# featureform/embeddinghub

Measured on AMD Instinct MI355X. Metric: kNN queries/sec at recall@10>=0.95, 10Mx768 cosine, batch=1024, higher is better.
Workload: dtype i8 filter -> f32 exact results; 1 GPU; 10000000x768 cosine (EHX-GAUSS-1), batch=1024, k=10, exact scan; rows=10000000, dims=768, batch=1024, k=10, rows_dtype=f32, world_size=1, parallelism=single GPU

## Files before the change

embeddinghub_amd/csrc/ehx_flat.cpp:

```cpp
#include "ehx_internal.h"

namespace ehx_impl {

ScanPlan plan_scan(uint32_t nq, uint32_t n_tiles, uint32_t k, int n_cus) {
  ScanPlan p;
  p.q_tiles = (nq + kTileQ - 1) / kTileQ;
  p.q_rows = p.q_tiles * kTileQ;
  p.n_tiles = n_tiles;
  p.kprime = k + 8;
  uint32_t chunks = (uint32_t)n_cus / p.q_tiles;
  if (chunks < 1) chunks = 1;
  if (chunks >= 8) chunks &= ~7u;
  if (chunks > p.n_tiles) chunks = p.n_tiles ? p.n_tiles : 1;
  p.n_chunks = chunks;
  p.tiles_per_chunk = p.n_tiles ? (p.n_tiles + chunks - 1) / chunks : 0;
  p.grid = p.q_tiles * p.n_chunks;
  p.xcd_map = (p.n_chunks % 8 == 0) ? 1u : 0u;
  return p;
}

std::vector<ScanPass> plan_cascade(uint32_t nq, uint32_t n_tiles, uint32_t k, int n_cus, uint64_t first_tiles, uint64_t growth) {
  std::vector<ScanPass> passes;
  uint64_t done = 0;
  for (uint64_t cum = first_tiles; cum * 2 < n_tiles; cum *= growth) {
// ... 60 lines not shown
                                  s->scr.dQgamma.p, s->scr.dQuv.p, st));
  if (n_pub == 0) {
    HIP_TRY(hipMemsetAsync(s->scr.dMerged.p, 0xFF, (size_t)p.q_rows * 64 * sizeof(uint64_t), st));
    if ((rc = clock.scan_begin(st)) || (rc = clock.scan_end(st))) return rc;
  } else {
    auto cascade = [&](auto& a, auto launch) -> int {
      for (size_t i = 0; i < passes.size(); ++i) {
        const bool last = i + 1 == passes.size();
        set_scan_pass(a, passes[i].plan, passes[i].tile0);
        HIP_TRY(launch(a, st));
        if (last && (rc = clock.scan_end(st))) return rc;
        HIP_TRY(launch_flat_merge(s->scr.dPart.p, (uint32_t)nq, passes[i].plan.n_chunks * lpc, p.kprime, s->scr.dMerged.p, st,
                                  lists_total, i > 0, last ? nullptr : (unsigned long long*)s->scr.dGthr.p));
      }
      return EHX_OK;
    };
    HIP_TRY(hipMemsetAsync(s->scr.dGthr.p, 0xFF, (size_t)p.q_rows * sizeof(uint64_t), st));
    if ((rc = clock.scan_begin(st))) return rc;
    if (f16) {
      ScanArgs16 h;
      scan_args_shared(h, s->scr.dCand.p, s->scr.dPart.p, s->scr.dScanErr.p, s->scr.dGthr.p, p, lists_total, n_pub);
      h.Q = s->scr.dQ16.p;
      h.X = s->f16.dX16.p;
      h.rowp = s->f16.dRowp16.p;
      h.qgamma = s->scr.dQgamma.p;
      h.eps = scan16_eps(s->dims);
      h.cos = s->metric == EHX_METRIC_COSINE;
      h.ld = s->ld16;
      if (sample) {
        ScanPlan sp = plan_scan((uint32_t)nq, kSampleTiles, k, E.n_cus);
        set_scan_pass(h, sp, 0);
        h.dump = s->scr.dSample.p;
        HIP_TRY(launch_flat_scan16(h, st));
        h.dump = nullptr;
        HIP_TRY(launch_sample_select(s->scr.dSample.p, kSampleTiles * kTileRows16, p.q_rows, (uint32_t)nq, p.kprime,
                                     (unsigned long long*)s->scr.dGthr.p, st));
      }
      if ((rc = cascade(h, launch_flat_scan16))) return rc;
    } else {
      ScanArgs a;
      scan_args_shared(a, s->scr.dCand.p, s->scr.dPart.p, s->scr.dScanErr.p, s->scr.dGthr.p, p, lists_total, n_pub);
      a.Q = s->scr.dQ.p;
      a.X = s->rows.dX.p;
      a.x_half = (uint32_t)s->x_half;
      a.rowp = s->rows.dRowp.p;
      a.ld = s->ld;
      if ((rc = cascade(a, launch_flat_scan8))) return rc;
    }
  }
  RerankArgs r;
  r.Q = s->scr.dQ.p;
  r.rows = rows_view(s, n_pub);
  r.merged = s->scr.dMerged.p;
  r.out_ids = d_ids;
  r.out_dist = d_dist;
  r.out_count = d_count;
  r.n_uncertified = s->scr.verdict.count.p;
  r.nq = (uint32_t)nq;
  r.k = k;
  r.kprime = p.kprime;
  if (f16) r.quv = s->scr.dQuv.p;
  r.max_sumsq = s->rows.dMaxSumsq.p;
  r.uncert_flags = s->scr.verdict.flags.p;
  HIP_TRY(launch_rerank(r, st));
  if ((rc = clock.finish(st))) return rc;
  s->n_rerank += (uint64_t)nq * p.kprime;
  return EHX_OK;
}

int resolve_engine(const ehx_space* s, uint64_t n_pub) {
  if (s->params.mode != EHX_MODE_FLAT || s->scan_sel == EHX_SCAN_F32 || n_pub == 0) return EHX_ENGINE_F32;
  if (s->scan_sel == EHX_SCAN_AUTO && s->has8 && s->h_unsafe8.load(std::memory_order_relaxed) == 0 && n_pub >= s->i8_min_rows)
    return EHX_ENGINE_I8;
  if (s->has16 && s->h_unsafe.load(std::memory_order_relaxed) == 0) return EHX_ENGINE_F16;
  return EHX_ENGINE_F32;
}

static int i8_diagnose(ehx_space::I8Set::Buffers& b, hipStream_t st, size_t nq, uint32_t k, uint32_t width,
                       const uint32_t* d_ovf, const float* d_dist) {
  HIP_TRY(hipStreamSynchronize(st));
  if (env().i8_count) {
    unsigned long long c[8] = {0};
    HIP_TRY(hipMemcpy(c, b.dCnt.p, sizeof(c), hipMemcpyDeviceToHost));
    fprintf(stderr, "[i8 count] tests %llu alarms %llu row-block alarms %llu trips %llu (cumulative)\n", c[0], c[1], c[2], c[3]);
  }
  if (env().i8_debug) {
    std::vector<uint32_t> fl(nq), ov(nq);
    std::vector<float4> qp(nq);
    std::vector<float2> uv(nq);
    std::vector<uint64_t> mg(nq * width);
    std::vector<float> od(nq * k);
    HIP_TRY(hipMemcpy(fl.data(), b.verdict.flags.p, nq * 4, hipMemcpyDeviceToHost));
    HIP_TRY(hipMemcpy(ov.data(), d_ovf, nq * 4, hipMemcpyDeviceToHost));
    HIP_TRY(hipMemcpy(qp.data(), b.dQp8.p, nq * sizeof(float4), hipMemcpyDeviceToHost));
    HIP_TRY(hipMemcpy(uv.data(), b.dQuv.p, nq * sizeof(float2), hipMemcpyDeviceToHost));
    HIP_TRY(hipMemcpy(mg.data(), b.dMerged8.p, nq * width * 8, hipMemcpyDeviceToHost));
    HIP_TRY(hipMemcpy(od.data(), d_dist, nq * k * 4, hipMemcpyDeviceToHost));
    int shown = 0;
    for (size_t q = 0; q < nq && shown < 6; ++q) {
      if (!fl[q]) continue;
      ++shown;
      auto S = [&](int i) { return mg[q * width + i] == ~0ull ? INFINITY : ordered_to_f32((uint32_t)(mg[q * width + i] >> 32)); };
      fprintf(stderr, "[i8 debug] q=%zu ovf=%u tmin=%g S[0]=%g S[63]=%g S[127]=%g S[255]=%g kth_dist=%g u=%g v=%g\n", q, ov[q],
              qp[q].w, S(0), S(63), S(127), S(255), od[q * k + k - 1], uv[q].x, uv[q].y);
    }
  }
  return EHX_OK;
}

static int flat_pass8(ehx_space* s, uint64_t n_pub, int set, hipStream_t st, size_t nq, const float* d_queries, uint32_t k,
                      uint64_t* d_ids, float* d_dist, uint32_t* d_count, uint32_t* kprime_used) {
  Engine& E = engine();
  ehx_space::I8Set& sc = s->i8set[set];
  const uint32_t n_tiles = (uint32_t)((n_pub + kTileRows16 - 1) / kTileRows16);
  const bool big = n_tiles >= 2048;
  const uint32_t growth = env().i8_growth ? env().i8_growth : (big ? 8u : 4u);
  const double safety = [] {
    return env().i8_safety;
  }();
  const int sync_mode = env().i8_sync;
  const bool use_sync = sync_mode > 0;
  constexpr uint32_t kSampleTiles = 8;
  const uint32_t width = s->i8_width.load(std::memory_order_relaxed);
  const long kprime_env = env().i8_kprime;
  uint32_t kp_auto = n_pub >= 4000000 ? 256u : 128u;
  if (s->dims <= 128) kp_auto = 64u;
  else if (s->dims < 512) kp_auto = 128u;
  if (s->dims >= 1024) kp_auto = width;
  const uint32_t kp_want = std::max(kp_auto, s->i8_kprime_min.load(std::memory_order_relaxed));
  const uint32_t kprime = kprime_env >= 64 ? (uint32_t)std::min<long>(kprime_env, (long)width) : std::min(kp_want, width);
  s->i8_kprime_last.store(kprime, std::memory_order_relaxed);
  *kprime_used = kprime;
  const uint32_t kFirstTiles = env().i8_first_tiles ? env().i8_first_tiles : (big ? 128u : 512u);
  const std::vector<ScanPass> passes = plan_cascade((uint32_t)nq, n_tiles, k, E.n_cus, kFirstTiles, growth);
  auto rank_after = [&](size_t i) -> uint32_t {
    if (i + 1 >= passes.size()) return kprime;
    const double f = (double)((uint64_t)(passes[i + 1].tile0) * kTileRows16) / (double)n_pub;
    return (uint32_t)std::min<double>(kprime, std::max<double>(16.0, std::ceil(kprime * f * safety)));
  };
  const uint64_t first_rows = (uint64_t)passes.front().plan.n_tiles * kTileRows16;
  const uint64_t first_keys_env = env().i8_first_keys;
  const uint64_t first_floor = first_keys_env ? first_keys_env : (big ? 64ull : std::min<uint64_t>(512, 2ull * kprime));
  const uint64_t first_keys = std::min<uint64_t>(
      2048, passes.size() == 1 ? 2ull * kprime : std::max<uint64_t>(first_floor, 2ull * rank_after(0)));
  const uint32_t sample_rank =
      (uint32_t)std::min<uint64_t>(64, std::max<uint64_t>(8, first_keys * kSampleTiles * kTileRows16 / first_rows));
  const ScanPlan p = passes.back().plan;
  test_pause();
  uint32_t grid_max = 0, chunks_max = 0;
  for (auto& ps : passes) {
    grid_max = std::max(grid_max, ps.plan.grid);
    chunks_max = std::max(chunks_max, ps.plan.n_chunks);
  }
  if (chunks_max > 256) return fail(EHX_EINTERNAL, "scan plan with %u chunks", chunks_max);
  int rc;
  ScanArgsI8 a;
  if ((rc = i8_scan_args(s, sc.buf, p, n_pub, &a))) return rc;
  if ((rc = sc.buf.dSample8.ensure((size_t)kSampleTiles * kTileRows16 * p.q_rows))) return rc;
  if ((rc = sc.buf.dMerged8.ensure((size_t)p.q_rows * width))) return rc;
  if ((rc = sc.buf.verdict.ensure(p.q_rows, ehx_space::I8Set::kStampWords))) return rc;
  constexpr uint32_t kTable = kBalanceMaxChunks + 1;
  std::vector<int> stamp_slot(passes.size(), -1);
  sc.n_stamped = 0;
  if (s->ld8 % 256u == 0u && !s->keyless) {
    const uint32_t min_tpc = s->i8_balance_min_tpc.load(std::memory_order_relaxed);
    uint32_t off = 0;
    for (size_t i = passes.size(); i-- > 0 && sc.n_stamped < ehx_space::I8Set::kStampedPasses;) {
// ... 334 lines not shown
```

embeddinghub_amd/csrc/k_flati8.hip:

```cpp
#include "ehx_env.h"
#include "ehx_kernels.h"
#include "k_scan_common.h"

namespace ehx {

typedef int i32x4 __attribute__((ext_vector_type(4)));

namespace {

constexpr uint32_t kRingI8 = 4;
constexpr uint32_t kRowBI8 = 64;
constexpr uint32_t kStageI8 = kTileRows16 * kRowBI8;
template <bool HALF>
struct I8L {
  static constexpr int kThreads = HALF ? 256 : 512;
  static constexpr uint32_t kWaves = HALF ? 4 : 8;
  static constexpr uint32_t kXStage = HALF ? kStageI8 / 2 : kStageI8;
  static constexpr uint32_t kXShift = HALF ? 13 : 14;
  static constexpr uint32_t kQSlots = HALF ? 2 : kRingI8;
  static constexpr uint32_t kStgCap = HALF ? 64 : 128;
  static constexpr uint32_t kRowpSlot = (HALF ? 128 : 256) * 16;
  static constexpr uint32_t kRowpWaves = HALF ? 2 : 4;
  static constexpr uint32_t kXOff = 0;
  static constexpr uint32_t kQOff = kRingI8 * kXStage;
  static constexpr uint32_t kRowpOff = kQOff + kQSlots * kStageI8;
  static constexpr uint32_t kQpOff = kRowpOff + 3 * kRowpSlot;
  static constexpr uint32_t kQinvOff = kQpOff + kTileQ * 16;
  static constexpr uint32_t kSyncOff = kQinvOff + kTileQ * 4;
  static constexpr uint32_t kCtxOff = kSyncOff + 256;
  static constexpr uint32_t kStgKeyOff = kCtxOff + 64;
  static constexpr uint32_t kStgQlOff = kStgKeyOff + kWaves * kStgCap * 8;
  static constexpr uint32_t kStgCntOff = kStgQlOff + kWaves * kStgCap * 4;
  static constexpr uint32_t kLdsBytes = kStgCntOff + 64;
};
static_assert(I8L<false>::kLdsBytes <= 160 * 1024, "LDS budget");
static_assert(I8L<true>::kLdsBytes <= 80 * 1024, "LDS budget: two half-tile workgroups per CU");
static_assert(I8L<false>::kQOff == 64 * 1024 && I8L<false>::kRowpOff == 128 * 1024, "layout of the full-tile kernel");
static_assert(kTileRows16 == 256 && kTileQ == 256, "kernel geometry is hard-wired");

#define EHX_MFMA_I8(A, B, C) __builtin_amdgcn_mfma_i32_16x16x64_i8((A), (B), (C), 0, 0, 0)

#ifndef EHX_I8_ABL
#define EHX_I8_ABL 0
#endif
#ifndef EHX_I8_COUNT
#define EHX_I8_COUNT 0
#endif
#ifndef EHX_I8_PRIO
#define EHX_I8_PRIO 1
#endif
#if EHX_I8_COUNT
#define EHX_CNT(I) do { if (lane == 0) atomicAdd((unsigned long long*)a.cand + (I), 1ull); } while (0)
#else
#define EHX_CNT(I) do { } while (0)
#endif

__device__ __forceinline__ void lds_barrier_i8() {
  __builtin_amdgcn_s_waitcnt(0xC07F);
  __builtin_amdgcn_s_barrier();
}

__device__ __forceinline__ float i8_score(const float4 P, const float4 qq, int v) {
  const float t = qq.x * (float)v;
  const float K = __builtin_fmaf(P.y, qq.z, __builtin_fmaf(P.z, qq.y, P.w));
  return __builtin_fmaf(P.x, t, K);
}

__device__ __forceinline__ float i8_alarm_k(const float4 tp, const float4 qq, const float qinv) {
  const float bg = tp.w * qq.z, ce = tp.y * qq.y;
  float num = bg - tp.z - ce - qq.w;
  num -= 1e-5f * (fabsf(bg) + tp.z + ce + fabsf(qq.w));
  if (!(num > 0.0f)) return -__builtin_inff();
  return num * qinv;
}

struct I8Ctx {
  uint64_t* pool;
  uint32_t* pool_cnt;
  uint32_t* ovf;
  const uint8_t* perm;
  const float4* rowp;
  uint32_t pool_cap;
  uint32_t n;
  uint32_t q_tile0;
  uint32_t allow_bits;
  const uint32_t* allow;
};
static_assert(sizeof(I8Ctx) <= 64, "I8Ctx slot");

constexpr int kMaskNone = 0, kMaskOne = 1, kMaskPerQuery = 2, kMaskLabel = 3;
template <bool HALF, int MASKED>
__device__ __attribute__((noinline)) void i8_flush_staging() {
  using L = I8L<HALF>;
  extern __shared__ __attribute__((aligned(16))) char smem[];
  const I8Ctx* ctx = (const I8Ctx*)(smem + L::kCtxOff);
  const int lane = threadIdx.x & 63, w = threadIdx.x >> 6;
  const uint64_t* keys = (const uint64_t*)(smem + L::kStgKeyOff) + (size_t)w * L::kStgCap;
  const uint32_t* qls = (const uint32_t*)(smem + L::kStgQlOff) + (size_t)w * L::kStgCap;
  const float4* qp_lds = (const float4*)(smem + L::kQpOff);
  uint32_t* cnt = (uint32_t*)(smem + L::kStgCntOff) + w;
  uint32_t n = *cnt;
  if (n > L::kStgCap) n = L::kStgCap;
  const uint32_t cap = ctx->pool_cap;
  for (uint32_t i = (uint32_t)lane; i < n; i += 64) {
    const uint64_t e = keys[i];
    const uint32_t posn = (uint32_t)e;
    const int v = (int)(uint32_t)(e >> 32);
    const uint32_t qloc = (uint32_t)(w & 3) * 64u + qls[i];
    const float4 qq = qp_lds[qloc];
    const float S = i8_score(ctx->rowp[posn], qq, v);
    if (!(S <= qq.w) || posn >= ctx->n) continue;
    const uint32_t id = (posn & 0xFFFFFF00u) | (uint32_t)ctx->perm[posn];
    if constexpr (MASKED == kMaskOne) {
      if (id >= ctx->allow_bits || !((ctx->allow[id >> 5] >> (id & 31u)) & 1u)) continue;
    }
    if constexpr (MASKED == kMaskPerQuery) {
      if (id >= ctx->allow_bits) continue;
      const uint32_t* block = ctx->allow;
      if (!((block[(size_t)block[ctx->q_tile0 + qloc] + (id >> 5)] >> (id & 31u)) & 1u)) continue;
    }
    if constexpr (MASKED == kMaskLabel) {
      if (id >= ctx->allow_bits) continue;
      const uint32_t* block = ctx->allow;
      if (block[(size_t)kLabelHead + id] != block[ctx->q_tile0 + qloc]) continue;
    }
    const uint64_t key = ((uint64_t)f32_to_ordered(S) << 32) | (uint64_t)id;
    const uint32_t q = ctx->q_tile0 + qloc;
    const uint32_t pos = atomicAdd(&ctx->pool_cnt[q], 1u);
    if (pos < cap) ctx->pool[(size_t)q * cap + pos] = key;
    else ctx->ovf[q] = 1u;
  }
  asm volatile("s_waitcnt vmcnt(0) lgkmcnt(0)" ::: "memory");
  if (lane == 0) *cnt = 0u;
  asm volatile("s_waitcnt lgkmcnt(0)" ::: "memory");
}

template <bool HALF, int MASKED>
__device__ __forceinline__ void i8_hit(int v, bool hi, uint32_t r_local, uint32_t tile_row0, int ql, int w, uint32_t& stg_n) {
  using L = I8L<HALF>;
  extern __shared__ __attribute__((aligned(16))) char smem[];
  const uint64_t m = __ballot(hi);
  if (m == 0ull) return;
  const uint32_t k = (uint32_t)__builtin_popcountll(m);
  uint32_t* cnt = (uint32_t*)(smem + L::kStgCntOff) + w;
  if (stg_n + k > L::kStgCap) {
    if ((threadIdx.x & 63) == 0) *cnt = stg_n;
    asm volatile("s_waitcnt lgkmcnt(0)" ::: "memory");
    i8_flush_staging<HALF, MASKED>();
    stg_n = 0u;
  }
  if (hi) {
    const uint32_t pos = stg_n + __builtin_amdgcn_mbcnt_hi((uint32_t)(m >> 32), __builtin_amdgcn_mbcnt_lo((uint32_t)m, 0u));
    uint64_t* keys = (uint64_t*)(smem + L::kStgKeyOff) + (size_t)w * L::kStgCap;
    uint32_t* qls = (uint32_t*)(smem + L::kStgQlOff) + (size_t)w * L::kStgCap;
    keys[pos] = ((uint64_t)(uint32_t)v << 32) | (uint64_t)(tile_row0 + r_local);
    qls[pos] = (uint32_t)ql;
  }
  stg_n += k;
}

}

size_t scan_i8_lds_bytes() { return I8L<false>::kLdsBytes; }

template <bool DUMP, bool REV, bool QRES = false, bool HALF = false, bool PAIR = false, int MASKED = kMaskNone, bool TAB = false>
__global__ __launch_bounds__(I8L<HALF>::kThreads, 2) void flat_scan_i8_kernel(const ScanArgsI8 a) {
  static_assert(!TAB || (REV && !DUMP && !QRES && !HALF && !PAIR && !MASKED), "TAB: the plain compile-time-slot scan only");
  static_assert(!QRES || (!REV && !DUMP), "QRES: the run-time-slot loop of the plain scan only");
  static_assert(!PAIR || (!REV && !DUMP && !QRES && !HALF), "PAIR: the run-time-slot loop of the plain scan, stages in pairs");
  static_assert(!HALF || QRES, "HALF: short rows, the query tile resident in LDS");
  static_assert(!MASKED || !DUMP, "MASKED: the flush of a collecting scan");
  using L = I8L<HALF>;
  extern __shared__ __attribute__((aligned(16))) char smem[];
  const int tid = threadIdx.x;
  const int lane = tid & 63;
  const int w = __builtin_amdgcn_readfirstlane(tid >> 6);
  const int j15 = lane & 15, qd = lane >> 4;

  uint32_t qt, chunk, half = 0u;
  {
    uint32_t b = blockIdx.x;
    if (a.xcd_map) {
      const uint32_t xcd = b & 7u;
      uint32_t slot = b >> 3;
      if constexpr (HALF) {
        half = slot & 1u;
        slot >>= 1;
      }
      qt = slot % a.q_tiles;
      chunk = xcd * (a.n_chunks >> 3) + slot / a.q_tiles;
    } else {
      if constexpr (HALF) {
        half = b & 1u;
        b >>= 1;
      }
      qt = b % a.q_tiles;
      chunk = b / a.q_tiles;
    }
    half = (uint32_t)__builtin_amdgcn_readfirstlane((int)half);
    qt = (uint32_t)__builtin_amdgcn_readfirstlane((int)qt);
    chunk = (uint32_t)__builtin_amdgcn_readfirstlane((int)chunk);
  }
  const int wr = HALF ? (int)half : (w >> 2), wc = w & 3;
  const uint32_t lrow0 = HALF ? 0u : (uint32_t)wr * 128u;
  float4* qp_lds = (float4*)(smem + L::kQpOff);
  float* qinv_lds = (float*)(smem + L::kQinvOff);

  if (tid < (int)kTileQ) {
    const size_t qg = (size_t)qt * kTileQ + tid;
    float4 qp = a.qparams[qg];
    qp.w = a.thr ? a.thr[qg] : __builtin_inff();
    qp_lds[tid] = qp;
    qinv_lds[tid] = qp.x > 0.0f ? (1.0f - 1e-5f) / qp.x : __builtin_inff();
  }
  if (tid < 64) ((uint32_t*)(smem + L::kSyncOff))[tid] = 0u;
  if (tid < 8) ((uint32_t*)(smem + L::kStgCntOff))[tid] = 0u;
  if (tid == 0) {
    I8Ctx* ctx = (I8Ctx*)(smem + L::kCtxOff);
    ctx->pool = a.pool;
    ctx->pool_cnt = a.pool_cnt;
    ctx->ovf = a.ovf;
    ctx->perm = a.perm;
    ctx->rowp = a.rowp;
    ctx->pool_cap = a.pool_cap;
    ctx->n = a.n;
    ctx->q_tile0 = qt * kTileQ;
    ctx->allow_bits = MASKED ? a.allow_bits : 0u;
    if constexpr (MASKED) ctx->allow = a.allow;
  }

  uint32_t tile_begin = a.tile0 + chunk * a.tiles_per_chunk;
  uint32_t tile_end = tile_begin + a.tiles_per_chunk;
  if (tile_end > a.tile0 + a.n_tiles) tile_end = a.tile0 + a.n_tiles;
  if constexpr (TAB) {
    if (a.bounds) {
      typedef const __attribute__((address_space(4))) uint32_t* cu32p;
      const uint64_t bv = (uint64_t)(a.bounds + chunk);
      const uint32_t blo = (uint32_t)__builtin_amdgcn_readfirstlane((int)(uint32_t)bv);
      const uint32_t bhi = (uint32_t)__builtin_amdgcn_readfirstlane((int)(uint32_t)(bv >> 32));
      const cu32p bp = (cu32p)(((uint64_t)bhi << 32) | blo);
      tile_begin = a.tile0 + bp[0];
      tile_end = a.tile0 + bp[1];
      if (tile_end > a.tile0 + a.n_tiles) tile_end = a.tile0 + a.n_tiles;
      if (tile_begin > tile_end) tile_begin = tile_end;
    }
  }
  const uint32_t my_tiles =
      (uint32_t)__builtin_amdgcn_readfirstlane((int)(tile_end > tile_begin ? tile_end - tile_begin : 0u));
  const uint32_t ktiles = a.ld / kRowBI8;

  const uint32_t voff = (uint32_t)lane * 16u;
  const uint32_t voff8 = voff + L::kXStage / 2;
  const size_t tile_bytes = (size_t)ktiles * kStageI8;
  const char* xsrc = (const char*)a.X + (size_t)tile_begin * tile_bytes + (size_t)half * L::kXStage * (HALF ? 1u : 0u) +
                     (size_t)w * 1024;
  const char* qbase = (const char*)a.Q + (size_t)qt * ((size_t)(ktiles + 3) * kStageI8) + (size_t)w * 1024;
  const char* qsrc = qbase;
  const uint32_t rpiece = (uint32_t)w & (L::kRowpWaves - 1u);
  const char* rsrc = (const char*)(a.rowp + (size_t)tile_begin * kTileRows16 + (HALF ? (size_t)half * 128u : 0u)) +
                     (size_t)rpiece * 1024;
  const uint32_t xdst = L::kXOff + (uint32_t)w * 1024u;
  const uint32_t qdst = L::kQOff + (uint32_t)w * 1024u;
  const uint32_t rdst = L::kRowpOff + rpiece * 1024u;

#define EHX_DMA(DST_BASE, DST_IMM, VOFF, SRC)                                                              \
  do {                                                                                                     \
    asm volatile("s_add_u32 m0, %0, %1\n\ts_nop 0\n\tglobal_load_lds_dwordx4 %2, %3"                       \
                 :                                                                                         \
                 : "s"(DST_BASE), "n"(DST_IMM), "v"(VOFF), "s"(SRC)                                        \
                 : "memory", "scc");                                                                       \
  } while (0)
#define EHX_DMA_RT(DST, VOFF, SRC)                                                       \
  do {                                                                                   \
    asm volatile("s_mov_b32 m0, %0\n\ts_nop 0\n\tglobal_load_lds_dwordx4 %1, %2"         \
                 :                                                                       \
                 : "s"(DST), "v"(VOFF), "s"(SRC)                                         \
                 : "memory");                                                            \
  } while (0)
#define EHX_DMA_X0(SLOT) EHX_DMA(xdst, (SLOT) * L::kXStage, voff, xsrc)
#define EHX_DMA_Q0(SLOT) EHX_DMA(qdst, (SLOT) * 16384, voff, qsrc)
#define EHX_DMA_X1(SLOT) EHX_DMA(xdst, (SLOT) * L::kXStage + L::kXStage / 2, voff8, xsrc)
#define EHX_DMA_Q1(SLOT)                               \
  do {                                                 \
    EHX_DMA(qdst, (SLOT) * 16384 + 8192, voff8, qsrc);  \
    xsrc += kStageI8;                                  \
    qsrc += kStageI8;                                  \
  } while (0)

  const uint32_t sw = scan8_swz((uint32_t)j15);
  uint32_t a_off = L::kXOff + (lrow0 + (uint32_t)j15) * kRowBI8 + (((uint32_t)qd) ^ sw) * 16u;
  uint32_t b_off = L::kQOff + (uint32_t)(wc * 64 + j15) * kRowBI8 + (((uint32_t)qd) ^ sw) * 16u;
  asm volatile("" : "+v"(a_off), "+v"(b_off));

  i32x4 acc[8][4];
#pragma unroll
  for (int rb = 0; rb < 8; ++rb)
#pragma unroll
    for (int cb = 0; cb < 4; ++cb)
#pragma unroll
      for (int r = 0; r < 4; ++r) acc[rb][cb][r] = 0;

  uint32_t rp_slot = 0u;
  uint32_t stg_n = 0u;
  typedef float f32x4 __attribute__((ext_vector_type(4)));
  typedef const __attribute__((address_space(4))) f32x4* cf4p;
  auto ldc = [](cf4p p, size_t i) -> float4 {
    const f32x4 v = p[i];
    return make_float4(v.x, v.y, v.z, v.w);
  };
  auto uniform_ptr = [](const void* p) -> cf4p {
    const uint64_t v = (uint64_t)p;
    const uint32_t lo = (uint32_t)__builtin_amdgcn_readfirstlane((int)(uint32_t)v);
    const uint32_t hi = (uint32_t)__builtin_amdgcn_readfirstlane((int)(uint32_t)(v >> 32));
    return (cf4p)(((uint64_t)hi << 32) | lo);
  };
  const uint32_t tile_par = my_tiles ? tile_begin : a.tile0;
  const cf4p tilep_c = uniform_ptr(a.tilep + tile_par);
  float4 tp_cur = ldc(tilep_c, 0);
  const cf4p tgp = uniform_ptr(a.tileg + (size_t)tile_par * 16 + (size_t)wr * 4);
  float4 tg_cur = ldc(tgp, 0);
  float4 tgb_cur = ldc(tgp, 2);
  auto epilogue = [&](uint32_t t) {
    const uint32_t tile = tile_begin + t;
    const uint32_t tile_row0 = tile * kTileRows16 + (HALF ? half * 128u : 0u);
    const uint32_t rp_off = L::kRowpOff + rp_slot * L::kRowpSlot;
    const float4* rp = (const float4*)(smem + rp_off);
    int lane_e = lane;
    asm volatile("" : "+v"(lane_e));
    const int j15 = lane_e & 15, qd = lane_e >> 4;
    const int col0 = wc * 64 + j15;
    const uint32_t rbase = lrow0 + 4u * (uint32_t)qd;
    if (DUMP) {
      const size_t n_s = (size_t)a.n_tiles * kTileRows16;
      float* const o0 = a.dump + scan8_dump_index((uint32_t)qt * kTileQ + (uint32_t)col0,
                                                  tile_row0 - a.tile0 * kTileRows16 + rbase, (uint32_t)n_s);
      const size_t cb_step = (n_s >> 4) << 8;
      const float4 q0 = qp_lds[col0], q1 = qp_lds[col0 + 16], q2 = qp_lds[col0 + 32], q3 = qp_lds[col0 + 48];
#pragma unroll
      for (int rb = 0; rb < 8; ++rb) {
        float4 s0, s1, s2, s3;
        float* const f0 = (float*)&s0;
        float* const f1 = (float*)&s1;
        float* const f2 = (float*)&s2;
        float* const f3 = (float*)&s3;
#pragma unroll
        for (int r = 0; r < 4; ++r) {
          const float4 P = rp[rbase + 16u * (uint32_t)rb + (uint32_t)r];
          f0[r] = i8_score(P, q0, acc[rb][0][r]);
          f1[r] = i8_score(P, q1, acc[rb][1][r]);
          f2[r] = i8_score(P, q2, acc[rb][2][r]);
          f3[r] = i8_score(P, q3, acc[rb][3][r]);
        }
        float* const o = o0 + 256 * rb;
        *(float4*)(o) = s0;
        *(float4*)(o + cb_step) = s1;
        *(float4*)(o + 2 * cb_step) = s2;
        *(float4*)(o + 3 * cb_step) = s3;
        asm volatile("" ::: "memory");
      }
      return;
    }
#if EHX_I8_ABL & 32
#pragma unroll
    for (int rb = 0; rb < 8; ++rb)
      asm volatile("" : : "v"(acc[rb][0]), "v"(acc[rb][1]), "v"(acc[rb][2]), "v"(acc[rb][3]));
    return;
#endif
    const float4 tp = tp_cur;
    const float4 tg = tg_cur;
    const float gm = qd == 0 ? tg.x : (qd == 1 ? tg.y : (qd == 2 ? tg.z : tg.w));
    const float rgm = (1.0f - 2e-6f) * __builtin_amdgcn_rcpf(gm);
    const float k_own = i8_alarm_k(tp, qp_lds[wc * 64 + lane_e], qinv_lds[wc * 64 + lane_e]);
    float g_own = 0.0f, dB = 0.0f;
    if (a.group_b) {
      const float4 tgb = tgb_cur;
      dB = i8_group_b_margin(qd == 0 ? tgb.x : (qd == 1 ? tgb.y : (qd == 2 ? tgb.z : tgb.w)), tp.w);
      g_own = fmaxf(qp_lds[wc * 64 + lane_e].z, 0.0f) * qinv_lds[wc * 64 + lane_e] * (1.0f - 1e-4f);
    }
#pragma unroll
    for (int cb = 0; cb < 4; ++cb) {
      float kq = __shfl(k_own, cb * 16 + j15, 64);
      if (a.group_b) kq = __builtin_fmaf(dB, __shfl(g_own, cb * 16 + j15, 64), kq);
      const int ti = (int)fminf(fmaxf(kq * rgm, -2.1e9f), 2.1e9f);
      int m8[8];
#pragma unroll
      for (int rb = 0; rb < 8; ++rb) {
        const i32x4 c = acc[rb][cb];
        m8[rb] = max(max(c[0], c[1]), max(c[2], c[3]));
      }
      const int im = max(max(max(m8[0], m8[1]), max(m8[2], m8[3])), max(max(m8[4], m8[5]), max(m8[6], m8[7])));
#if EHX_I8_ABL & 2
      if (im >= ti) asm volatile("" ::: "memory");
      continue;
#endif
      EHX_CNT(0);
      if (!__any(im >= ti)) continue;
      EHX_CNT(1);
      const int ql = cb * 16 + j15;
      uint32_t pend = 0u;
#pragma unroll
      for (int rb = 7; rb >= 0; --rb) {
        uint32_t nib = 0u;
        if (__any(m8[rb] >= ti)) {
          EHX_CNT(2);
          const i32x4 c = acc[rb][cb];
#pragma unroll
          for (int r = 0; r < 4; ++r) nib |= (c[r] >= ti) ? (1u << r) : 0u;
        }
        pend = (pend << 4) | nib;
      }
      while (__any(pend != 0u)) {
        EHX_CNT(3);
        const bool hi = pend != 0u;
        int v = 0;
        uint32_t r_local = rbase;
        if (hi) {
          const int b = __builtin_ctz(pend);
          pend &= pend - 1u;
          i32x4 c4 = acc[0][cb];
#pragma unroll
          for (int rb = 1; rb < 8; ++rb) {
            const bool pick = (b >> 2) == rb;
            const i32x4 o = acc[rb][cb];
            c4[0] = pick ? o[0] : c4[0];
            c4[1] = pick ? o[1] : c4[1];
            c4[2] = pick ? o[2] : c4[2];
            c4[3] = pick ? o[3] : c4[3];
          }
          const int r = b & 3;
          v = r == 0 ? c4[0] : (r == 1 ? c4[1] : (r == 2 ? c4[2] : c4[3]));
          r_local = rbase + 16u * (uint32_t)(b >> 2) + (uint32_t)r;
        }
        i8_hit<HALF, MASKED>(v, hi, r_local, tile_row0, ql, w, stg_n);
      }
    }
  };

  uint32_t* const sync_ctr = (a.sync && a.sync_tol > 0u && a.xcd_map && a.q_tiles > 1 && REV && a.q_tiles <= 4)
                                 ? a.sync + chunk * 4u
                                 : nullptr;
  bool sync_on = sync_ctr != nullptr && !DUMP && !HALF;
  const uint32_t sync_m0 = L::kSyncOff;

  __syncthreads();
#if EHX_I8_PRIO
  {
    uint32_t hwid_p;
    asm volatile("s_getreg_b32 %0, hwreg(HW_REG_HW_ID)" : "=s"(hwid_p));
    if (hwid_p & 1u) __builtin_amdgcn_s_setprio(1);
  }
#endif
  if constexpr (HALF) {
    if (a.skew && my_tiles >= 16u) {
      uint32_t hwid;
      asm volatile("s_getreg_b32 %0, hwreg(HW_REG_HW_ID)" : "=s"(hwid));
      if (hwid & 1u) {
        for (uint32_t i = 32; i <= a.skew; i += 32) __builtin_amdgcn_s_sleep(32);
        for (uint32_t i = 0; i < (a.skew & 31u); ++i) __builtin_amdgcn_s_sleep(1);
      }
    }
  }
  if constexpr (TAB) {
    if (a.stamps) {
      if (tid == 0) a.stamps[2u * blockIdx.x] = wall_clock64();
      asm volatile("s_waitcnt vmcnt(0)" ::: "memory");
    }
  }
  if (my_tiles > 0) {
  if (DUMP && w < (int)L::kRowpWaves) EHX_DMA(rdst, 0, voff, rsrc);
  constexpr int kStageWait = QRES ? 4 : 8;
  if constexpr (QRES) {
    for (uint32_t ks = 0; ks < ktiles; ++ks) {
      const uint32_t qd0 = qdst + (ks << 14);
      constexpr uint32_t kQStep = HALF ? 4096u : 8192u;
#pragma unroll
      for (uint32_t pc = 0; pc < 16u / L::kWaves; ++pc) {
        const uint32_t qdp = qd0 + pc * kQStep, vo = voff + pc * kQStep;
        asm volatile("s_mov_b32 m0, %0\n\ts_nop 0\n\tglobal_load_lds_dwordx4 %1, %2" : : "s"(qdp), "v"(vo), "s"(qsrc) : "memory");
      }
      qsrc += kStageI8;
    }
    EHX_DMA_X0(0); EHX_DMA_X1(0); xsrc += kStageI8;
    EHX_DMA_X0(1); EHX_DMA_X1(1); xsrc += kStageI8;
    EHX_DMA_X0(2); EHX_DMA_X1(2); xsrc += kStageI8;
  } else {
    EHX_DMA_X0(0); EHX_DMA_Q0(0); EHX_DMA_X1(0); EHX_DMA_Q1(0);
    EHX_DMA_X0(1); EHX_DMA_Q0(1); EHX_DMA_X1(1); EHX_DMA_Q1(1);
    EHX_DMA_X0(2); EHX_DMA_Q0(2); EHX_DMA_X1(2); EHX_DMA_Q1(2);
  }
  wait_vmcnt<kStageWait>();
  lds_barrier_i8();
#if EHX_I8_ABL & 4
  wait_vmcnt<0>();
#define EHX_SDMA(DST, VOFF, SRC) do { } while (0)
#else
#define EHX_SDMA(DST, VOFF, SRC) EHX_DMA_RT(DST, VOFF, SRC)
#endif

  i32x4 fa[8], fb0[4], fb1[4];
#pragma unroll
  for (int rb = 0; rb < 8; ++rb) fa[rb] = *(const i32x4*)(smem + a_off + rb * 1024);
#pragma unroll
  for (int cb = 0; cb < 4; ++cb) fb0[cb] = *(const i32x4*)(smem + b_off + cb * 1024);

#if EHX_I8_ABL & 8
#define EHX_FR(P) fa[0]
#else
#define EHX_FR(P) (*(const i32x4*)(P))
#endif
#define EHX_MF(B, RB, CB) acc[RB][CB] = EHX_MFMA_I8(fa[RB], B[CB], acc[RB][CB])
  const i32x4 zero4 = {0, 0, 0, 0};
#define EHX_MFZ(B, RB, CB) acc[RB][CB] = EHX_MFMA_I8(fa[RB], B[CB], zero4)
#define EHX_SB() __builtin_amdgcn_sched_barrier(0)
#if EHX_I8_ABL & 16
#define EHX_STAGE_BARRIER() do { } while (0)
#else
#define EHX_STAGE_BARRIER() lds_barrier_i8()
// ... 177 lines not shown
    xsrc += kStageI8;                                                                                                 \
    tile_done();                                                                                                      \
  } while (0)
        uint32_t left = my_tiles;
#pragma unroll 1
        for (; left >= 2u; left -= 2u) {
          EHX_TILE2_CT(0);
          EHX_TILE2_CT(2);
        }
        if (left) EHX_TILE2_CT(0);
#undef EHX_TILE2_CT
#undef EHX_NODMA
        st = total_stages;
      }
    }
    if constexpr (PAIR) {
      {
#define EHX_RT_STAGE2(M0, BC, BN)                                                               \
  do {                                                                                          \
    const uint32_t sn = ((slot + 1u) & 3u) << L::kXShift, sd = ((slot + 3u) & 3u) << L::kXShift; \
    const uint32_t dx0 = xdst + sd, dq0 = qdst + sd;                                            \
    const uint32_t an_ = a_off + sn, bn_ = b_off + sn;                                          \
    EHX_STAGE16_BODY(M0, BC, BN, an_, bn_, EHX_RT_DX0, EHX_RT_DQ0, EHX_RT_DX1, EHX_RT_DQ1);     \
    xsrc += kStageI8;                                                                           \
    qsrc += kStageI8;                                                                           \
    slot = (slot + 1u) & 3u;                                                                    \
    ++st;                                                                                       \
  } while (0)
#pragma unroll 1
        while (st < total_stages) {
          if (ks == 0u) EHX_RT_STAGE2(EHX_MFZ, fb0, fb1);
          else EHX_RT_STAGE2(EHX_MF, fb0, fb1);
          EHX_RT_STAGE2(EHX_MF, fb1, fb0);
          ks += 2u;
          if (ks == ktiles) {
            ks = 0;
            tile_done();
          }
        }
#undef EHX_RT_STAGE2
      }
    }
    if constexpr (!PAIR) {
#pragma unroll 1
      while (st < total_stages) {
        if (ks == 0u)
          EHX_RT_STAGE(EHX_STAGE16_BODY(EHX_MFZ, fb0, fb1, an_, bn_, EHX_RT_DX0, EHX_RT_DQ0, EHX_RT_DX1, EHX_RT_DQ1));
        else
          EHX_RT_STAGE(EHX_STAGE16_BODY(EHX_MF, fb0, fb1, an_, bn_, EHX_RT_DX0, EHX_RT_DQ0, EHX_RT_DX1, EHX_RT_DQ1));
        if (++ks == ktiles) {
          ks = 0;
          tile_done();
        }
      }
    }
#undef EHX_RT_STAGE
#undef EHX_RT_DX0
#undef EHX_RT_DQ0
#undef EHX_RT_DX1
#undef EHX_RT_DQ1
  }
  }
#undef EHX_MF
#undef EHX_SB
#undef EHX_FR
#undef EHX_SDMA
#undef EHX_DMA_RT
#undef EHX_SDMA_X0
#undef EHX_SDMA_Q0
#undef EHX_SDMA_X1
#undef EHX_SDMA_Q1
#undef EHX_STAGE16_CT
#undef EHX_STAGE16_BODY
#undef EHX_STAGE_BARRIER
#undef EHX_MFZ
#undef EHX_DMA_X0
#undef EHX_DMA_Q0
#undef EHX_DMA_X1
#undef EHX_DMA_Q1
#undef EHX_DMA

  asm volatile("s_waitcnt vmcnt(0) lgkmcnt(0)" ::: "memory");
  if (DUMP) return;
  if (lane == 0) ((uint32_t*)(smem + L::kStgCntOff))[w] = stg_n;
  asm volatile("s_waitcnt lgkmcnt(0)" ::: "memory");
  i8_flush_staging<HALF, MASKED>();
  if constexpr (TAB) {
    if (a.stamps) {
      __syncthreads();
      if (tid == 0) a.stamps[2u * blockIdx.x + 1u] = wall_clock64();
    }
  }
}

hipError_t launch_flat_scan_i8(const ScanArgsI8& a, hipStream_t st) {
  static DynLdsAttr attr;
  const void* fns[] = {(const void*)flat_scan_i8_kernel<false, true>, (const void*)flat_scan_i8_kernel<false, false>,
                       (const void*)flat_scan_i8_kernel<true, true>, (const void*)flat_scan_i8_kernel<true, false>,
                       (const void*)flat_scan_i8_kernel<false, false, true>,
                       (const void*)flat_scan_i8_kernel<false, false, true, true>,
                       (const void*)flat_scan_i8_kernel<false, false, false, false, true>,
                       (const void*)flat_scan_i8_kernel<false, true, false, false, false, true>,
                       (const void*)flat_scan_i8_kernel<false, false, false, false, false, true>,
                       (const void*)flat_scan_i8_kernel<false, false, true, false, false, true>,
                       (const void*)flat_scan_i8_kernel<false, false, true, true, false, true>,
                       (const void*)flat_scan_i8_kernel<false, false, false, false, true, true>,
                       (const void*)flat_scan_i8_kernel<false, true, false, false, false, kMaskPerQuery>,
                       (const void*)flat_scan_i8_kernel<false, false, false, false, false, kMaskPerQuery>,
                       (const void*)flat_scan_i8_kernel<false, false, true, false, false, kMaskPerQuery>,
                       (const void*)flat_scan_i8_kernel<false, false, true, true, false, kMaskPerQuery>,
                       (const void*)flat_scan_i8_kernel<false, false, false, false, true, kMaskPerQuery>,
                       (const void*)flat_scan_i8_kernel<false, true, false, false, false, kMaskLabel>,
                       (const void*)flat_scan_i8_kernel<false, false, false, false, false, kMaskLabel>,
                       (const void*)flat_scan_i8_kernel<false, false, true, false, false, kMaskLabel>,
                       (const void*)flat_scan_i8_kernel<false, false, true, true, false, kMaskLabel>,
                       (const void*)flat_scan_i8_kernel<false, false, false, false, true, kMaskLabel>,
                       (const void*)flat_scan_i8_kernel<false, true, false, false, false, kMaskNone, true>};
  if (hipError_t e = attr.ensure(fns, (int)(sizeof(fns) / sizeof(fns[0])), I8L<false>::kLdsBytes); e != hipSuccess) return e;
  if (a.ld == 0 || a.ld % kRowBI8) return hipErrorInvalidValue;
  const uint32_t grid = a.q_tiles * a.n_chunks;
  const bool rev = a.ld % (4 * kRowBI8) == 0;
#define EHX_LAUNCH_I8(D, R) \
  hipLaunchKernelGGL((flat_scan_i8_kernel<D, R>), dim3(grid), dim3(I8L<false>::kThreads), I8L<false>::kLdsBytes, st, a)
  const bool qres_on = env().i8_qres;
  if (a.allow) {
    if (a.dump) return hipErrorInvalidValue;
#define EHX_LAUNCH_I8_MASKED(M)                                                                                              \
  do {                                                                                                                       \
    if (rev)                                                                                                                 \
      hipLaunchKernelGGL((flat_scan_i8_kernel<false, true, false, false, false, M>), dim3(grid), dim3(I8L<false>::kThreads), \
                         I8L<false>::kLdsBytes, st, a);                                                                      \
    else if (qres_on && env().i8_half && a.ld <= 2 * kRowBI8)                                                                \
      hipLaunchKernelGGL((flat_scan_i8_kernel<false, false, true, true, false, M>), dim3(2 * grid),                          \
                         dim3(I8L<true>::kThreads), I8L<true>::kLdsBytes, st, a);                                            \
    else if (qres_on && a.ld <= 4 * kRowBI8)                                                                                 \
      hipLaunchKernelGGL((flat_scan_i8_kernel<false, false, true, false, false, M>), dim3(grid), dim3(I8L<false>::kThreads), \
                         I8L<false>::kLdsBytes, st, a);                                                                      \
    else if ((a.ld / kRowBI8) % 2u == 0u)                                                                                    \
      hipLaunchKernelGGL((flat_scan_i8_kernel<false, false, false, false, true, M>), dim3(grid), dim3(I8L<false>::kThreads), \
                         I8L<false>::kLdsBytes, st, a);                                                                      \
    else                                                                                                                     \
      hipLaunchKernelGGL((flat_scan_i8_kernel<false, false, false, false, false, M>), dim3(grid),                            \
                         dim3(I8L<false>::kThreads), I8L<false>::kLdsBytes, st, a);                                          \
  } while (0)
    if (a.allow_label && (a.allow_per_query || a.q_tiles * 256u > kLabelHead)) return hipErrorInvalidValue;
    if (a.allow_label) EHX_LAUNCH_I8_MASKED(kMaskLabel);
    else if (a.allow_per_query) EHX_LAUNCH_I8_MASKED(kMaskPerQuery);
    else EHX_LAUNCH_I8_MASKED(kMaskOne);
#undef EHX_LAUNCH_I8_MASKED
  } else if (a.dump) {
    if (rev) EHX_LAUNCH_I8(true, true);
    else EHX_LAUNCH_I8(true, false);
  } else {
    const bool half_on = env().i8_half;
    if (rev && (a.bounds || a.stamps))
      hipLaunchKernelGGL((flat_scan_i8_kernel<false, true, false, false, false, kMaskNone, true>), dim3(grid),
                         dim3(I8L<false>::kThreads), I8L<false>::kLdsBytes, st, a);
    else if (a.bounds || a.stamps) return hipErrorInvalidValue;
    else if (rev) EHX_LAUNCH_I8(false, true);
    else if (qres_on && half_on && a.ld <= 2 * kRowBI8)
      hipLaunchKernelGGL((flat_scan_i8_kernel<false, false, true, true>), dim3(2 * grid), dim3(I8L<true>::kThreads),
                         I8L<true>::kLdsBytes, st, a);
    else if (qres_on && a.ld <= 4 * kRowBI8)
      hipLaunchKernelGGL((flat_scan_i8_kernel<false, false, true>), dim3(grid), dim3(I8L<false>::kThreads), I8L<false>::kLdsBytes, st, a);
    else if ((a.ld / kRowBI8) % 2u == 0u)
      hipLaunchKernelGGL((flat_scan_i8_kernel<false, false, false, false, true>), dim3(grid), dim3(I8L<false>::kThreads),
                         I8L<false>::kLdsBytes, st, a);
    else EHX_LAUNCH_I8(false, false);
// ... 7 lines not shown
```

Before: 169,700 queries/s.

## Stage alarmed i8 accumulator groups in LDS and expand them in bulk

Replaces the per-lane serial extraction of threshold hits from the int8 MFMA accumulators, which selected one hit at a time with a chain of selects under a divergent loop, with a two-level scheme. Each alarming lane now dumps its whole 32-value accumulator column plus header into an LDS group buffer that reuses the row-parameter region. A noinline expander later turns these groups into staged keys two groups per wave pass using ballot and mbcnt. This is meant to cut divergent scalar work and register pressure in the hot scan loop. In exchange it adds LDS writes of 144 bytes per alarming lane, extra drain and flush points, and a larger LDS layout.

```diff
diff --git a/embeddinghub_amd/csrc/ehx_flat.cpp b/embeddinghub_amd/csrc/ehx_flat.cpp
--- a/embeddinghub_amd/csrc/ehx_flat.cpp
+++ b/embeddinghub_amd/csrc/ehx_flat.cpp
@@ -166,7 +166,8 @@
   if (env().i8_count) {
     unsigned long long c[8] = {0};
     HIP_TRY(hipMemcpy(c, b.dCnt.p, sizeof(c), hipMemcpyDeviceToHost));
-    fprintf(stderr, "[i8 count] tests %llu alarms %llu row-block alarms %llu trips %llu (cumulative)\n", c[0], c[1], c[2], c[3]);
+    fprintf(stderr, "[i8 count] tests %llu alarms %llu staged groups %llu values at their level %llu keys %llu (cumulative)\n",
+            c[0], c[1], c[2], c[3], c[4]);
   }
   if (env().i8_debug) {
     std::vector<uint32_t> fl(nq), ov(nq);
diff --git a/embeddinghub_amd/csrc/k_flati8.hip b/embeddinghub_amd/csrc/k_flati8.hip
--- a/embeddinghub_amd/csrc/k_flati8.hip
+++ b/embeddinghub_amd/csrc/k_flati8.hip
@@ -11,6 +11,7 @@
 constexpr uint32_t kRingI8 = 4;
 constexpr uint32_t kRowBI8 = 64;
 constexpr uint32_t kStageI8 = kTileRows16 * kRowBI8;
+constexpr uint32_t kGrpBytes = 16 + 32 * 4;
 template <bool HALF>
 struct I8L {
   static constexpr int kThreads = HALF ? 256 : 512;
@@ -19,19 +20,23 @@
   static constexpr uint32_t kXShift = HALF ? 13 : 14;
   static constexpr uint32_t kQSlots = HALF ? 2 : kRingI8;
   static constexpr uint32_t kStgCap = HALF ? 64 : 128;
+  static constexpr uint32_t kGrpCap = 12;
   static constexpr uint32_t kRowpSlot = (HALF ? 128 : 256) * 16;
   static constexpr uint32_t kRowpWaves = HALF ? 2 : 4;
   static constexpr uint32_t kXOff = 0;
   static constexpr uint32_t kQOff = kRingI8 * kXStage;
   static constexpr uint32_t kRowpOff = kQOff + kQSlots * kStageI8;
-  static constexpr uint32_t kQpOff = kRowpOff + 3 * kRowpSlot;
+  static constexpr uint32_t kGrpOff = kRowpOff;
+  static constexpr uint32_t kRowpGrpBytes = 3 * kRowpSlot > kWaves * kGrpCap * kGrpBytes ? 3 * kRowpSlot : kWaves * kGrpCap * kGrpBytes;
+  static constexpr uint32_t kQpOff = kRowpOff + kRowpGrpBytes;
   static constexpr uint32_t kQinvOff = kQpOff + kTileQ * 16;
   static constexpr uint32_t kSyncOff = kQinvOff + kTileQ * 4;
   static constexpr uint32_t kCtxOff = kSyncOff + 256;
   static constexpr uint32_t kStgKeyOff = kCtxOff + 64;
   static constexpr uint32_t kStgQlOff = kStgKeyOff + kWaves * kStgCap * 8;
   static constexpr uint32_t kStgCntOff = kStgQlOff + kWaves * kStgCap * 4;
-  static constexpr uint32_t kLdsBytes = kStgCntOff + 64;
+  static constexpr uint32_t kCandOff = kStgCntOff + 64;
+  static constexpr uint32_t kLdsBytes = kCandOff + 16;
 };
 static_assert(I8L<false>::kLdsBytes <= 160 * 1024, "LDS budget");
 static_assert(I8L<true>::kLdsBytes <= 80 * 1024, "LDS budget: two half-tile workgroups per CU");
@@ -51,8 +56,13 @@
 #endif
 #if EHX_I8_COUNT
 #define EHX_CNT(I) do { if (lane == 0) atomicAdd((unsigned long long*)a.cand + (I), 1ull); } while (0)
+#define EHX_CNT_LDS(I, N)                                                                                                 \
+  do {                                                                                                                    \
+    if (lane == 0) atomicAdd(*(unsigned long long**)(smem + L::kCandOff) + (I), (unsigned long long)(N));                 \
+  } while (0)
 #else
 #define EHX_CNT(I) do { } while (0)
+#define EHX_CNT_LDS(I, N) do { } while (0)
 #endif
 
 __device__ __forceinline__ void lds_barrier_i8() {
@@ -129,6 +139,9 @@
     const uint32_t pos = atomicAdd(&ctx->pool_cnt[q], 1u);
     if (pos < cap) ctx->pool[(size_t)q * cap + pos] = key;
     else ctx->ovf[q] = 1u;
+#if EHX_I8_COUNT
+    atomicAdd(*(unsigned long long**)(smem + L::kCandOff) + 4, 1ull);
+#endif
   }
   asm volatile("s_waitcnt vmcnt(0) lgkmcnt(0)" ::: "memory");
   if (lane == 0) *cnt = 0u;
@@ -136,27 +149,98 @@
 }
 
 template <bool HALF, int MASKED>
-__device__ __forceinline__ void i8_hit(int v, bool hi, uint32_t r_local, uint32_t tile_row0, int ql, int w, uint32_t& stg_n) {
+__device__ __attribute__((noinline)) void i8_expand_groups() {
+  using L = I8L<HALF>;
+  extern __shared__ __attribute__((aligned(16))) char smem[];
+  const int lane = threadIdx.x & 63, w = threadIdx.x >> 6;
+  uint32_t* cnt = (uint32_t*)(smem + L::kStgCntOff) + w;
+  const uint32_t gw = (uint32_t)__builtin_amdgcn_readfirstlane((int)cnt[8]);
+  uint32_t ng = gw & 0xFFFFu, g0 = gw >> 16;
+  if (ng > L::kGrpCap) ng = L::kGrpCap;
+  uint32_t nk = (uint32_t)__builtin_amdgcn_readfirstlane((int)cnt[0]);
+  if (nk > L::kStgCap) nk = L::kStgCap;
+  const char* grp = smem + L::kGrpOff + (uint32_t)w * (L::kGrpCap * kGrpBytes);
+  uint64_t* keys = (uint64_t*)(smem + L::kStgKeyOff) + (size_t)w * L::kStgCap;
+  uint32_t* qls = (uint32_t*)(smem + L::kStgQlOff) + (size_t)w * L::kStgCap;
+  const uint32_t j = (uint32_t)lane & 31u;
+  uint32_t left = 0u;
+  for (; g0 < ng; g0 += 2u) {
+    const uint32_t g = g0 + ((uint32_t)lane >> 5);
+    bool hi = false;
+    int v = 0;
+    uint32_t posn = 0u, ql = 0u;
+    if (g < ng) {
+      const char* e = grp + g * kGrpBytes;
+      const uint32_t* h = (const uint32_t*)e;
+      v = *(const int*)(e + 16u + 4u * j);
+      hi = v >= (int)h[2];
+      posn = h[0] + 16u * (j >> 2) + (j & 3u);
+      ql = h[1];
+    }
+    const uint64_t m = __ballot(hi);
+    const uint32_t k = (uint32_t)__builtin_popcountll(m);
+    if (nk + k > L::kStgCap) {
+      left = (g0 << 16) | ng;
+      break;
+    }
+    EHX_CNT_LDS(3, k);
+    if (hi) {
+      const uint32_t pos = nk + __builtin_amdgcn_mbcnt_hi((uint32_t)(m >> 32), __builtin_amdgcn_mbcnt_lo((uint32_t)m, 0u));
+      keys[pos] = ((uint64_t)(uint32_t)v << 32) | (uint64_t)posn;
+      qls[pos] = ql;
+    }
+    nk += k;
+  }
+  if (lane == 0) {
+    cnt[0] = nk;
+    cnt[8] = left;
+  }
+  asm volatile("s_waitcnt lgkmcnt(0)" ::: "memory");
+}
+
+template <bool HALF, int MASKED>
+__device__ __forceinline__ void i8_drain_groups(uint32_t ng, int w) {
+  using L = I8L<HALF>;
+  extern __shared__ __attribute__((aligned(16))) char smem[];
+  uint32_t* gcnt = (uint32_t*)(smem + L::kStgCntOff) + 8 + w;
+  if ((threadIdx.x & 63) == 0) *gcnt = ng;
+  for (;;) {
+    asm volatile("s_waitcnt lgkmcnt(0)" ::: "memory");
+    i8_expand_groups<HALF, MASKED>();
+    if (__builtin_amdgcn_readfirstlane((int)*gcnt) == 0) return;
+    i8_flush_staging<HALF, MASKED>();
+  }
+}
+
+template <bool HALF, int MASKED>
+__device__ __forceinline__ void i8_stage_groups(const i32x4 (&c)[8], bool hi, uint32_t posn0, int ql, int ti, int w, uint32_t& grp_n) {
   using L = I8L<HALF>;
   extern __shared__ __attribute__((aligned(16))) char smem[];
   const uint64_t m = __ballot(hi);
-  if (m == 0ull) return;
   const uint32_t k = (uint32_t)__builtin_popcountll(m);
-  uint32_t* cnt = (uint32_t*)(smem + L::kStgCntOff) + w;
-  if (stg_n + k > L::kStgCap) {
-    if ((threadIdx.x & 63) == 0) *cnt = stg_n;
-    asm volatile("s_waitcnt lgkmcnt(0)" ::: "memory");
-    i8_flush_staging<HALF, MASKED>();
-    stg_n = 0u;
-  }
-  if (hi) {
-    const uint32_t pos = stg_n + __builtin_amdgcn_mbcnt_hi((uint32_t)(m >> 32), __builtin_amdgcn_mbcnt_lo((uint32_t)m, 0u));
-    uint64_t* keys = (uint64_t*)(smem + L::kStgKeyOff) + (size_t)w * L::kStgCap;
-    uint32_t* qls = (uint32_t*)(smem + L::kStgQlOff) + (size_t)w * L::kStgCap;
-    keys[pos] = ((uint64_t)(uint32_t)v << 32) | (uint64_t)(tile_row0 + r_local);
-    qls[pos] = (uint32_t)ql;
-  }
-  stg_n += k;
+  const uint32_t rank =
+      hi ? __builtin_amdgcn_mbcnt_hi((uint32_t)(m >> 32), __builtin_amdgcn_mbcnt_lo((uint32_t)m, 0u)) : 0x7FFFFFFFu;
+  uint32_t done = 0u;
+  for (;;) {
+    const uint32_t room = L::kGrpCap - grp_n;
+    const uint32_t idx = rank - done;
+    if (idx < room) {
+      char* e = smem + L::kGrpOff + ((uint32_t)w * L::kGrpCap + grp_n + idx) * kGrpBytes;
+      ((uint32_t*)e)[0] = posn0;
+      ((int*)e)[1] = ql;
+      ((int*)e)[2] = ti;
+#pragma unroll
+      for (int rb = 0; rb < 8; ++rb) *(i32x4*)(e + 16 + 16 * rb) = c[rb];
+    }
+    if (k - done < room) {
+      grp_n += k - done;
+      return;
+    }
+    i8_drain_groups<HALF, MASKED>(L::kGrpCap, w);
+    grp_n = 0u;
+    done += room;
+    if (done == k) return;
+  }
 }
 
 }
@@ -214,7 +298,10 @@
     qinv_lds[tid] = qp.x > 0.0f ? (1.0f - 1e-5f) / qp.x : __builtin_inff();
   }
   if (tid < 64) ((uint32_t*)(smem + L::kSyncOff))[tid] = 0u;
-  if (tid < 8) ((uint32_t*)(smem + L::kStgCntOff))[tid] = 0u;
+  if (tid < 16) ((uint32_t*)(smem + L::kStgCntOff))[tid] = 0u;
+#if EHX_I8_COUNT
+  if (tid == 0) *(unsigned long long**)(smem + L::kCandOff) = (unsigned long long*)a.cand;
+#endif
   if (tid == 0) {
     I8Ctx* ctx = (I8Ctx*)(smem + L::kCtxOff);
     ctx->pool = a.pool;
@@ -301,7 +388,7 @@
       for (int r = 0; r < 4; ++r) acc[rb][cb][r] = 0;
 
   uint32_t rp_slot = 0u;
-  uint32_t stg_n = 0u;
+  uint32_t grp_n = 0u;
   typedef float f32x4 __attribute__((ext_vector_type(4)));
   typedef const __attribute__((address_space(4))) f32x4* cf4p;
   auto ldc = [](cf4p p, size_t i) -> float4 {
@@ -396,43 +483,14 @@
       EHX_CNT(0);
       if (!__any(im >= ti)) continue;
       EHX_CNT(1);
-      const int ql = cb * 16 + j15;
-      uint32_t pend = 0u;
-#pragma unroll
-      for (int rb = 7; rb >= 0; --rb) {
-        uint32_t nib = 0u;
-        if (__any(m8[rb] >= ti)) {
-          EHX_CNT(2);
-          const i32x4 c = acc[rb][cb];
-#pragma unroll
-          for (int r = 0; r < 4; ++r) nib |= (c[r] >= ti) ? (1u << r) : 0u;
-        }
-        pend = (pend << 4) | nib;
-      }
-      while (__any(pend != 0u)) {
-        EHX_CNT(3);
-        const bool hi = pend != 0u;
-        int v = 0;
-        uint32_t r_local = rbase;
-        if (hi) {
-          const int b = __builtin_ctz(pend);
-          pend &= pend - 1u;
-          i32x4 c4 = acc[0][cb];
-#pragma unroll
-          for (int rb = 1; rb < 8; ++rb) {
-            const bool pick = (b >> 2) == rb;
-            const i32x4 o = acc[rb][cb];
-            c4[0] = pick ? o[0] : c4[0];
-            c4[1] = pick ? o[1] : c4[1];
-            c4[2] = pick ? o[2] : c4[2];
-            c4[3] = pick ? o[3] : c4[3];
-          }
-          const int r = b & 3;
-          v = r == 0 ? c4[0] : (r == 1 ? c4[1] : (r == 2 ? c4[2] : c4[3]));
-          r_local = rbase + 16u * (uint32_t)(b >> 2) + (uint32_t)r;
-        }
-        i8_hit<HALF, MASKED>(v, hi, r_local, tile_row0, ql, w, stg_n);
-      }
+      const i32x4 c8[8] = {acc[0][cb], acc[1][cb], acc[2][cb], acc[3][cb], acc[4][cb], acc[5][cb], acc[6][cb], acc[7][cb]};
+#if EHX_I8_COUNT
+      {
+        const unsigned long long n_grp = (unsigned long long)__builtin_popcountll(__ballot(im >= ti));
+        if (lane == 0) atomicAdd((unsigned long long*)a.cand + 2, n_grp);
+      }
+#endif
+      i8_stage_groups<HALF, MASKED>(c8, im >= ti, tile_row0 + rbase, cb * 16 + j15, ti, w, grp_n);
     }
   };
 
@@ -776,8 +834,7 @@
 
   asm volatile("s_waitcnt vmcnt(0) lgkmcnt(0)" ::: "memory");
   if (DUMP) return;
-  if (lane == 0) ((uint32_t*)(smem + L::kStgCntOff))[w] = stg_n;
-  asm volatile("s_waitcnt lgkmcnt(0)" ::: "memory");
+  i8_drain_groups<HALF, MASKED>(grp_n, w);
   i8_flush_staging<HALF, MASKED>();
   if constexpr (TAB) {
     if (a.stamps) {
```

Result: no change. 169,600 queries/s (-0.1%).
